# MasterVVK/qwen3-tts-axera-russian

Measured on AMD Instinct MI355X. Metric: 12Hz codec-tokens/s (codec frames/s, 16 codes each) + RTF, Qwen3-TTS-0.6B, higher is better.
Workload: dtype f16 weights/KV, f32 accumulate (talker+CP); vocoder exact fp32 (f32 MFMA); 1 GPU; configs[2]/[3]: batch=32 mixed ru/en prompts per GPU, 64 frames/utterance/step (prefill + hipGraph decode loop), utterance-sharded DP over 1 GPU(s); batch_per_gpu=32

## Files before the change

qwen3_tts_axera_russian_amd/build.py:

```python
from __future__ import annotations

import os
import shutil
import subprocess
import sys

HERE = os.path.dirname(os.path.abspath(__file__))
CSRC = os.path.join(HERE, "csrc")
LIB = os.path.join(HERE, "lib")
SOURCES = ["q3_common.cpp", "q3_formats.cpp", "q3_kernels.hip", "q3_model.hip", "q3_talker_api.hip", "q3_cp_api.hip",
           "q3_engine.hip", "q3_voc.hip", "q3_enc.hip", "q3_text_api.hip"]
TEST_SOURCES = ["q3_test_api.hip"]
ARCH = os.environ.get("Q3_OFFLOAD_ARCH", "gfx950")
EXTRA = os.environ.get("Q3_EXTRA_HIPCC_FLAGS", "-mllvm -amdgpu-kernarg-preload-count=16").split()


def _newer(dst: str, srcs) -> bool:
    if not os.path.exists(dst):
        return False
    t = os.path.getmtime(dst)
    return all(os.path.getmtime(s) <= t for s in srcs)


NO_SPILL = ("resunit_kernel", "linear_kernelILi1ELi1E", "linear_kernelILi1ELi2E", "linear_kernelILi2ELi1E",
            "linear_kernelILi2ELi2E", "attn_kernel", "attn_short_kernel", "cp_argmax_kernel", "talker_sample_kernel",
            "voc_attn_incr_kernel", "voc_incr_prepend_kernel", "voc_incr_emit_kernel")


def kernel_resources(lib_path: str):
    import re
    import struct
    import tempfile
    readelf = "/opt/rocm/lib/llvm/bin/llvm-readelf"
    d = open(lib_path, "rb").read()
    res = {}
    i = d.find(b"__CLANG_OFFLOAD_BUNDLE__")
    while i >= 0:
        n = struct.unpack_from("<Q", d, i + 24)[0]
        off = i + 32
        for _ in range(n):
            o, sz, ts = struct.unpack_from("<QQQ", d, off)
            off += 24
            triple = d[off:off + ts].decode()
            off += ts
            if ARCH in triple and sz:
                with tempfile.NamedTemporaryFile(suffix=".elf") as f:
                    f.write(d[i + o:i + o + sz])
                    f.flush()
# ... 85 lines not shown
```

qwen3_tts_axera_russian_amd/csrc/q3_cp.h:

```cpp
#pragma once
#include "q3_model.h"

namespace q3 {

struct CpFrameIO {
    int* codes = nullptr;
    const int* n_frames = nullptr;
    int frame_cap = 1;
    float* fb_h = nullptr;
    float* fb_ssq = nullptr;
    half_t* fb_xh = nullptr;
    const float* fb_gamma = nullptr;
    const float* pad_embed = nullptr;
    float temperature = 0.f;
    int top_k = 50;
    unsigned long long seed = 0;
    const unsigned long long* seed_ptr = nullptr;
    const int* forced = nullptr;
    const SlotParams* slots = nullptr;
};

int cp_seed_row0(const Work& w, int R, int row0 = 0, int R_total = 0);
int cp_frame(hipStream_t s, const Model& m, Work& w, KVCache& kv, int R, const CpFrameIO& io, int row0 = 0,
             int R_total = 0);

}
```

qwen3_tts_axera_russian_amd/csrc/q3_cp_api.hip:

```cpp
#include "../../include/qwen3tts_cp.h"
#include "q3_cp.h"

namespace q3 {

static bool two_row_enabled() {
    static const bool on = !(getenv("Q3_CP_TWO_ROW") && atoi(getenv("Q3_CP_TWO_ROW")) == 0);
    return on;
}

int cp_seed_row0(const Work& w, int R, int row0, int R_total) {
    (void)R;
    (void)row0;
    if (R_total <= 0) R_total = R;
    const int B16 = (R_total + 15) / 16 * 16;
    const bool two = two_row_enabled() && 2 * B16 <= w.max_rows;
    return two ? B16 : 0;
}

int cp_frame(hipStream_t s, const Model& m, Work& w, KVCache& kv, int R, const CpFrameIO& io, int row0, int R_total) {
    const ModelCfg& c = m.cfg;
    if (R_total <= 0) R_total = R;
    const int H = c.hidden, G = c.cp_groups;
    const int seed0 = cp_seed_row0(w, R, row0, R_total);
    RowMap rm;
    rm.slot_base = 0;
    rm.slot_stride = 1;
    rm.pos_stride = 0;
    if (seed0 > 0 && (row0 != 0 || R_total != R)) {
        RowMap r0;
        r0.slot_base = -seed0;
        r0.slot_stride = 1;
        r0.pos_base = 0;
        r0.pos_stride = 0;
        r0.same_slot_rows = true;
        if (run_stack(s, m, m.cp, w, kv, R, r0, 256, seed0 + row0)) return -1;
        if (launch_gather_embed(s, m.talker_emb, c.talker_vocab, H, io.codes, 0, io.n_frames, io.frame_cap, 0, w.h, w.ssq, R,
                                row0, R_total, io.forced, w.xh, m.cp.L[0].in_ln))
            return -1;
        RowMap r1 = rm;
        r1.pos_base = 1;
        r1.same_slot_rows = true;
        if (run_stack(s, m, m.cp, w, kv, R, r1, 256, row0)) return -1;
    } else if (seed0 > 0) {
        const int R16 = seed0;
        if (w.map_R16 != R16) {
            std::vector<int> slot(2 * R16), pos(2 * R16);
            for (int i = 0; i < 2 * R16; i++) {
                slot[i] = i % R16;
                pos[i] = i < R16 ? 1 : 0;
            }
            Q3_HIP(hipMemcpyAsync(w.map_slot, slot.data(), sizeof(int) * 2 * R16, hipMemcpyHostToDevice, s), -1);
            Q3_HIP(hipMemcpyAsync(w.map_pos, pos.data(), sizeof(int) * 2 * R16, hipMemcpyHostToDevice, s), -1);
            Q3_HIP(hipStreamSynchronize(s), -1);
            w.map_R16 = R16;
        }
        if (launch_gather_embed(s, m.talker_emb, c.talker_vocab, H, io.codes, 0, io.n_frames, io.frame_cap, 0, w.h, w.ssq, R,
                                row0, R_total, io.forced, w.xh, m.cp.L[0].in_ln))
            return -1;
        RowMap r2;
        r2.slot = w.map_slot;
        r2.pos = w.map_pos;
        r2.same_slot_rows = true;
        r2.valid_mod = R16;
        r2.valid_n = R;
        if (run_stack(s, m, m.cp, w, kv, R16 + R, r2, 256, 0)) return -1;
    } else {
        rm.pos_base = 0;
        if (run_stack(s, m, m.cp, w, kv, R, rm, 256, row0)) return -1;
        if (launch_gather_embed(s, m.talker_emb, c.talker_vocab, H, io.codes, 0, io.n_frames, io.frame_cap, 0, w.h, w.ssq, R,
                                row0, R_total, io.forced, w.xh, m.cp.L[0].in_ln))
            return -1;
        rm.pos_base = 1;
        if (run_stack(s, m, m.cp, w, kv, R, rm, 256, row0)) return -1;
    }
    const bool qkv_tab = m.cp_qkv_serves(R);
    for (int g = 0; g < G; g++) {
        if (g > 0) {
            rm.pos_base = g + 1;
            rm.skip_qkv0 = qkv_tab;
            if (run_stack(s, m, m.cp, w, kv, R, rm, 256, row0)) return -1;
        }
        LinArgs a;
        a.wp = m.cp_head[g].wp;
        a.N = c.cp_vocab;
        a.K = H;
        a.M = row0 + R;
        a.m_begin = row0;
// ... 234 lines not shown
```

qwen3_tts_axera_russian_amd/csrc/q3_engine.hip:

```cpp
#include "../../include/qwen3tts_engine.h"
#include "q3_cp.h"

#include <algorithm>
#include <chrono>
#include <cmath>

using namespace q3;

namespace {

struct Engine {
    Model* m = nullptr;
    int max_batch = 0, n_ctx = 0, max_frames = 0;
    hipStream_t s = nullptr;
    KVCache kv_t, kv_c;
    Work wt, wc;
    int prefill_rows = 0;
    int *d_slot = nullptr, *d_pos = nullptr;
    int* d_tiles = nullptr;
    int *d_iota = nullptr;
    int *d_past = nullptr, *d_npast = nullptr, *d_ntext = nullptr, *d_done = nullptr, *d_nframes = nullptr;
    int *d_pos0 = nullptr, *d_posdec = nullptr, *d_lastrow = nullptr;
    int* d_codes = nullptr;
    int* d_forced = nullptr;
// ... 72 lines not shown
    sa.R = R;
    sa.row0 = row0;
    sa.R_total = e->B;
    sa.audio_vocab = m.cfg.cp_vocab;
    sa.eos = m.cfg.codec_eos;
    sa.past = e->d_past;
    sa.n_past = e->d_npast;
    sa.n_text = e->d_ntext;
    sa.done = e->d_done;
    sa.codes = e->d_codes;
    sa.n_frames = e->d_nframes;
    sa.frame_cap = e->max_frames;
    sa.pos0 = e->d_pos0;
    sa.pos = e->d_posdec;
    sa.ignore_eos = e->ignore_eos;
    sa.max_frames = e->cap_frames;
    sa.temperature = e->t_temp;
    sa.top_k = e->t_top_k;
    sa.top_p = e->t_top_p;
    sa.seed = e->seed;
    sa.seed_ptr = e->d_seed;
    sa.forced = e->forced_on ? e->d_forced : nullptr;
    sa.slots = e->slot_mode ? e->d_slots : nullptr;
    if (launch_talker_sample(st, sa)) return -1;
    CpFrameIO io;
    io.codes = e->d_codes;
    io.n_frames = e->d_nframes;
    io.frame_cap = e->max_frames;
    io.fb_h = e->wt.h;
    io.fb_ssq = e->wt.ssq;
    io.fb_xh = e->wt.xh;
    io.fb_gamma = m.talker.L[0].in_ln;
    io.pad_embed = e->d_pad;
    io.temperature = e->c_temp;
    io.top_k = e->c_top_k;
    io.seed = e->seed ^ 0x5851F42D4C957F2Dull;
    io.seed_ptr = e->d_seed;
    io.forced = e->forced_on ? e->d_forced : nullptr;
    io.slots = e->slot_mode ? e->d_slots : nullptr;
    if (cp_frame(st, m, e->wc, e->kv_c, R, io, row0, e->B)) return -1;
    RowMap rm;
    rm.slot_base = 0;
    rm.slot_stride = 1;
    rm.pos = e->d_posdec;
    rm.rows_total = e->B;
    if (run_stack(st, m, m.talker, e->wt, e->kv_t, R, rm, 1024, row0)) return -1;
    return talker_tail(e, st, row0, R);
}

int n_chains_eff(const Engine* e) {
    const int nc = e->n_chains < 1 ? 1 : e->n_chains;
    return (nc > 1 && e->B % (16 * nc) == 0) ? nc : 1;
}

void chain_rows(const Engine* e, int c, int& row0, int& R) {
    const int nc = n_chains_eff(e);
    row0 = 0;
    for (int i = 0; i < c; i++) row0 += e->B / nc + (i < e->B % nc ? 1 : 0);
    R = e->B / nc + (c < e->B % nc ? 1 : 0);
}

bool make_stream(const Engine* e, hipStream_t* st) {
// ... 20 lines not shown
        chain_rows(e, c, row0, R);
        if (frame_chain(e, chain_stream(e, c), row0, R)) return -1;
    }
    return 0;
}

int fork_chains(Engine* e) {
    const int nc = n_chains_eff(e);
    if (nc == 1) return 0;
    Q3_HIP(hipEventRecord(e->ev_fork, e->s), -1);
    for (int c = 0; c < nc; c++) Q3_HIP(hipStreamWaitEvent(e->cs[c], e->ev_fork, 0), -1);
    return 0;
}
int join_chains(Engine* e) {
    const int nc = n_chains_eff(e);
    if (nc == 1) return 0;
    for (int c = 0; c < nc; c++) {
        Q3_HIP(hipEventRecord(e->ev_join[c], e->cs[c]), -1);
        Q3_HIP(hipStreamWaitEvent(e->s, e->ev_join[c], 0), -1);
    }
    return 0;
}

}

extern "C" {

void q3e_free(void* ee) {
    Engine* e = (Engine*)ee;
    if (!e) return;
    if (e->s) hipStreamSynchronize(e->s);
    for (auto& g : e->graph) g.reset();
    kv_free(e->kv_t);
    kv_free(e->kv_c);
    work_free(e->wt);
    work_free(e->wc);
    void* ps[] = {e->d_tiles, e->d_slot, e->d_pos,  e->d_iota,   e->d_past,    e->d_npast, e->d_ntext, e->d_done,
                  e->d_nframes, e->d_pos0, e->d_posdec, e->d_lastrow, e->d_codes, e->d_pad, e->d_forced, e->d_seed, e->d_slots};
    for (void* p : ps)
        if (p) hipFree(p);
    if (e->h_done) hipHostFree(e->h_done);
    if (e->h_read) hipHostFree(e->h_read);
    for (int c = 0; c < 8; c++) {
        if (e->cs[c]) hipStreamDestroy(e->cs[c]);
        if (e->ev_join[c]) hipEventDestroy(e->ev_join[c]);
    }
// ... 597 lines not shown
```

qwen3_tts_axera_russian_amd/csrc/q3_kernels.h:

```cpp
#pragma once
#include "q3_common.h"

namespace q3 {

enum { PRO_F16 = 0, PRO_NORM = 1 };
enum { EPI_STORE = 0, EPI_RESID = 1, EPI_SWIGLU = 2 };

struct LinArgs {
    int tl_node = -1;
    const half_t* wp = nullptr;
    int N = 0, K = 0, M = 0;
    int m_begin = 0;
    int swap_grid = 0;
    int nt = 0;
    const half_t* x16 = nullptr;
    const float* ssq = nullptr;
    int ssq_parts = 0;
    float eps = 1e-6f;
    float* y = nullptr;
    int ldy = 0;
    float* h_out = nullptr;
    float* ssq_out = nullptr;
    half_t* xh_out = nullptr;
    const float* gamma = nullptr;
// ... 7 lines not shown

enum { ATTN_FUSED = 0, ATTN_PREP = 1, ATTN_ATTEND = 2 };
struct AttnArgs {
    int tl_node = -1;
    float* qkv = nullptr;
    int ld = 0, R = 0, row0 = 0;
    const float* q_norm = nullptr;
    const float* k_norm = nullptr;
    float eps = 1e-6f;
    const float* rope_cos = nullptr;
    const float* rope_sin = nullptr;
    const int* slot = nullptr;
    const int* pos = nullptr;
    int slot_base = 0, slot_stride = 0, pos_base = 0, pos_stride = 0;
    half_t* kc = nullptr;
    half_t* vc = nullptr;
    int n_ctx = 0, n_kv = 0, n_heads = 0;
    half_t* out = nullptr;
    float scale = 0.f;
    int threads = 256;
    int valid_mod = 0, valid_n = 0;
    const int* tiles = nullptr;
    int n_tiles = 0;
};
int launch_attn(hipStream_t s, const AttnArgs& a, int mode);

int launch_ssq_rows(hipStream_t s, const float* rows, float* h, float* ssq, int R, int H, half_t* xh = nullptr,
                    const float* gamma = nullptr, int dst_row0 = 0);

struct FinalNormArgs {
    int tl_node = -1;
    const float* h = nullptr;
    const float* ssq = nullptr;
    int ssq_parts = 0;
    const float* gamma = nullptr;
    float eps = 1e-6f;
    int R = 0, H = 0, row0 = 0;
    const int* row_map = nullptr;
    int src_off = 0;
    float* out_f32 = nullptr;
    half_t* out_f16 = nullptr;
    float* out_copy = nullptr;
    float* out_copy_ssq = nullptr;
    int out_copy_row_off = 0;
    half_t* out_copy_xh = nullptr;
    const float* out_copy_gamma = nullptr;
};
int launch_final_norm(hipStream_t s, const FinalNormArgs& a);
// ... 17 lines not shown
struct TalkerSampleArgs {
    int tl_node = -1;
    const float* logits = nullptr;
    int V = 0, R = 0, row0 = 0, R_total = 0;
    int audio_vocab = 2048, eos = 2150;
    int* past = nullptr;
    int* n_past = nullptr;
    const int* n_text = nullptr;
    int* done = nullptr;
    int* codes = nullptr;
    int* n_frames = nullptr;
    int frame_cap = 0;
    const int* pos0 = nullptr;
    int* pos = nullptr;
    int ignore_eos = 0;
    int max_frames = 0;
    float rep_penalty = 1.2f;
    float temperature = 0.f, top_p = 0.95f;
    int top_k = 50;
    unsigned long long seed = 0;
    const unsigned long long* seed_ptr = nullptr;
    const int* forced = nullptr;
    const SlotParams* slots = nullptr;
};
int launch_talker_sample(hipStream_t s, const TalkerSampleArgs& a);

struct CpArgmaxArgs {
    int tl_node = -1;
    const float* logits = nullptr;
    int V = 0, R = 0, H = 0, row0 = 0, R_total = 0;
    int group = 0;
    int* codes = nullptr;
    const int* n_frames = nullptr;
    int frame_cap = 0;
    const float* next_table = nullptr;
    float* h_out = nullptr;
    float* ssq_out = nullptr;
    half_t* xh_out = nullptr;
    const float* gamma_next = nullptr;
    const float* next_qkv = nullptr;
    float* qkv_out = nullptr;
    int qkv_ld = 0;
    const float* talker_emb = nullptr;
    int talker_vocab = 0;
    const float* const* cp_tables = nullptr;
    const float* pad_embed = nullptr;
// ... 18 lines not shown
```

qwen3_tts_axera_russian_amd/csrc/q3_kernels.hip:

```cpp
#include "q3_kernels.h"

namespace q3 {

typedef _Float16 h8 __attribute__((ext_vector_type(8)));
typedef float f4 __attribute__((ext_vector_type(4)));

#ifdef Q3_TIMELINE
__device__ unsigned long long* g_tl = nullptr;
__device__ unsigned int g_tl_idx = 0;
__device__ unsigned int g_tl_cap = 0;
__device__ int g_skip = 0;
__device__ unsigned long long* g_ph = nullptr;
struct TlScope {
    unsigned int slot = 0xffffffffu;
    int id;
    __device__ __forceinline__ TlScope(int id_) : id(id_) {
        if (blockIdx.x == 0 && blockIdx.y == 0 && threadIdx.x == 0 && g_tl) {
            slot = atomicAdd(&g_tl_idx, 1u);
            if (slot < g_tl_cap) g_tl[2 * slot] = (wall_clock64() << 8) | (unsigned)id;
        }
    }
    __device__ __forceinline__ ~TlScope() {
        if (slot < g_tl_cap) g_tl[2 * slot + 1] = wall_clock64();
    }
};
__device__ unsigned long long* g_tl2 = nullptr;
__device__ int* g_tl2_kind = nullptr;
constexpr int TL2_MAXB = 1024;
struct TlScope2 {
    unsigned long long t0;
    int node, kind;
    __device__ __forceinline__ TlScope2(int n, int k) : node(n), kind(k) { t0 = wall_clock64(); }
    __device__ __forceinline__ ~TlScope2() {
        if (g_tl2 && node >= 0 && threadIdx.x == 0) {
            const unsigned b = blockIdx.x + gridDim.x * blockIdx.y;
            if (b < TL2_MAXB) {
                g_tl2[((size_t)node * TL2_MAXB + b) * 2] = t0;
                g_tl2[((size_t)node * TL2_MAXB + b) * 2 + 1] = wall_clock64();
            }
            if (b == 0 && g_tl2_kind) g_tl2_kind[node] = kind;
        }
    }
};
#define Q3_TL(id)      \
    if (g_skip) return; \
    TlScope2 tl_scope2_(a.tl_node, id); \
    TlScope tl_scope_(id)
#define Q3_PH(n)                                                                                       \
    do {                                                                                               \
        if (tl_scope_.slot < g_tl_cap && g_ph) g_ph[(size_t)tl_scope_.slot * 8 + (n)] = wall_clock64(); \
    } while (0)
#else
#ifndef Q3_WAVE_PRIO
#define Q3_WAVE_PRIO 3
#endif
#if Q3_WAVE_PRIO > 0
#define Q3_TL(id) __builtin_amdgcn_s_setprio(Q3_WAVE_PRIO)
#else
#define Q3_TL(id)
#endif
#define Q3_PH(n)
#endif

#define Q3_FETCH_ARGS(...) asm volatile("" ::__VA_ARGS__)

__device__ __forceinline__ int uniform_load(const int* p) {
    return *(const __attribute__((address_space(4))) int*)p;
}

__device__ __forceinline__ float wave_sum(float v) {
#pragma unroll
    for (int o = 32; o > 0; o >>= 1) v += __shfl_xor(v, o, 64);
    return v;
}
__device__ __forceinline__ float wave_max(float v) {
#pragma unroll
    for (int o = 32; o > 0; o >>= 1) v = fmaxf(v, __shfl_xor(v, o, 64));
    return v;
}
__device__ __forceinline__ half_t sat_half(float x) {
    return (half_t)fminf(fmaxf(x, -65504.f), 65504.f);
}
constexpr float NORM_PRE = 0.0625f, NORM_POST = 16.0f;
// ... 1165 lines not shown
#pragma unroll
    for (int e4 = 0; e4 < NE; e4 += 4) {
        const float4 t4 = *(const float4*)(&sc[hh][e4]);
        sv[e4] = t4.x;
        sv[e4 + 1] = t4.y;
        sv[e4 + 2] = t4.z;
        sv[e4 + 3] = t4.w;
    }
    float m = -INFINITY;
#pragma unroll
    for (int e = 0; e < NE; e++) m = fmaxf(m, e <= T ? sv[e] : -INFINITY);
    float L = 0.f, o = 0.f;
#pragma unroll
    for (int e = 0; e < NE; e++) {
        const float p = e <= T ? __expf(sv[e] - m) : 0.f;
        const float vf = e <= T ? (float)vs[e][d] : 0.f;
        L += p;
        o += p * vf;
    }
    Q3_PH(3);
    a.out[frag_idx(r, (2 * g + hh) * D + d, a.n_heads * D)] = sat_half(o / L);
}

__global__ void __launch_bounds__(256) attn_tile_mfma_kernel(AttnArgs a) {
    constexpr int D = 128, QP = 136, VP = 72, CH = 64;
    constexpr float LO = 2048.0f, ILO = 1.0f / 2048.0f;
    Q3_TL(35);
    const int g = blockIdx.y, tid = threadIdx.x, lane = tid & 63, w = tid >> 6;
    const int c = lane & 15, q4 = lane >> 4;
    int row0, nrows, slot, pos0;
    if (a.tiles) {
        const int4 t = *(const int4*)(a.tiles + 4 * blockIdx.x);
        row0 = t.x; nrows = t.y; slot = t.z; pos0 = t.w;
    } else {
        row0 = a.row0 + blockIdx.x * 16;
        nrows = a.R - blockIdx.x * 16 < 16 ? a.R - blockIdx.x * 16 : 16;
        slot = a.slot_base;
        pos0 = a.pos_base + blockIdx.x * 16;
    }
    extern __shared__ __attribute__((aligned(16))) char smem[];
    half_t* qh = (half_t*)smem;
    half_t* ql = qh + 32 * QP;
    half_t* ks = ql + 32 * QP;
    half_t* vs = ks + CH * QP;
    half_t* ph = vs + CH * QP;
    half_t* pl = ph + 32 * VP;
// ... 192 lines not shown
        return 0;
    }
    int threads = a.threads;
    const int fit = 65536 / (a.R * a.n_kv);
    if (threads > fit) threads = fit / 64 * 64;
    if (threads < 256) threads = 256;
    if (threads > 1024) threads = 1024;
    const size_t lds = ((size_t)(threads / 64) * (4 + 2 * 128)) * sizeof(float);
    AttnArgs a2 = a;
    a2.tl_node = tl_next_node();
    dim3 grid(a.R, a.n_kv);
#define Q3_ATTN(MODE_)                                                                                   \
    {                                                                                                    \
        if (threads <= 256)                                                                              \
            hipLaunchKernelGGL((attn_kernel<MODE_, 8>), grid, dim3(256), mode == ATTN_PREP ? 0 : lds, s, a2); \
        else                                                                                             \
            hipLaunchKernelGGL((attn_kernel<MODE_, 4>), grid, dim3(mode == ATTN_PREP ? 256 : threads),   \
                               mode == ATTN_PREP ? 0 : lds, s, a2);                                      \
    }
    if (mode == ATTN_FUSED) Q3_ATTN(ATTN_FUSED)
    else if (mode == ATTN_PREP) Q3_ATTN(ATTN_PREP)
    else Q3_ATTN(ATTN_ATTEND)
#undef Q3_ATTN
    Q3_HIP(hipGetLastError(), -1);
    return 0;
}

__device__ __forceinline__ void block_argmax(float& v, int& idx, float* sv, int* si) {
#pragma unroll
    for (int o = 32; o > 0; o >>= 1) {
        const float ov = __shfl_xor(v, o, 64);
        const int oi = __shfl_xor(idx, o, 64);
        if (ov > v || (ov == v && oi < idx)) {
            v = ov;
            idx = oi;
        }
    }
    const int w = threadIdx.x >> 6, nw = blockDim.x >> 6;
    if ((threadIdx.x & 63) == 0) {
        sv[w] = v;
        si[w] = idx;
    }
    __syncthreads();
    v = sv[0];
    idx = si[0];
    for (int i = 1; i < nw; i++)
// ... 160 lines not shown
    __syncthreads();
    return chosen;
}

__device__ __forceinline__ SlotParams uniform_slot(const SlotParams* p, int r) {
    static_assert(sizeof(SlotParams) % 4 == 0, "SlotParams is read as words");
    constexpr int NW = (int)(sizeof(SlotParams) / 4);
    const __attribute__((address_space(4))) int* q = (const __attribute__((address_space(4))) int*)(p + r);
    int w[NW];
#pragma unroll
    for (int i = 0; i < NW; i++) w[i] = q[i];
    SlotParams sp;
    __builtin_memcpy(&sp, w, sizeof(sp));
    return sp;
}

template <bool SLOTS>
__device__ __forceinline__ void talker_sample_row(const TalkerSampleArgs& a) {
    Q3_TL(42);
    __shared__ float sv[16];
    __shared__ int si[16];
    __shared__ int win[32];
    __shared__ int nwin;
    const int r = a.row0 + blockIdx.x;
    const int RT = a.R_total > 0 ? a.R_total : a.R;
    const int np = uniform_load(a.n_past + r);
    const int nt = uniform_load(a.n_text + r);
    const bool was_done = uniform_load(a.done + r) != 0;
    float temperature = a.temperature, top_p = a.top_p;
    int top_k = a.top_k, max_frames = a.max_frames;
    if constexpr (SLOTS) {
        const SlotParams sp = uniform_slot(a.slots, r);
        temperature = sp.t_temp;
        top_p = sp.t_top_p;
        top_k = sp.t_top_k;
        max_frames = sp.max_frames;
    }
    if (threadIdx.x == 0) nwin = np < 30 ? np : 30;
    if (threadIdx.x < 30 && threadIdx.x < np) {
        win[threadIdx.x] = a.past[r * 32 + ((np - 1 - threadIdx.x) & 31)];
    }
    __syncthreads();
    double progress = 0.0;
    float boost = 0.f;
    bool force_eos = false;
    if (nt > 0) {
// ... 44 lines not shown
        if (bidx >= a.V) bidx = a.eos;
    }
    if (threadIdx.x == 0) {
        int code = bidx;
        if (force_eos && !a.ignore_eos) code = a.eos;
        bool fin = was_done || code == a.eos || code >= a.audio_vocab || (max_frames > 0 && np >= max_frames);
        const int f = a.n_frames[r];
        if (!SLOTS || !fin || f <= a.frame_cap) a.n_frames[r] = f + 1;
        const bool keep = f < a.frame_cap;
        int* fc = a.codes + ((size_t)(keep ? f : 0) * RT + r) * 16;
        int used = code;
        if (a.forced && keep && !fin) {
            const int fz = a.forced[((size_t)f * RT + r) * 16];
            if (fz >= 0) used = fz;
        }
        if (fin || !keep) {
            a.done[r] = 1;
            if (keep) fc[0] = -1;
        } else {
            fc[0] = code;
            a.past[r * 32 + (np & 31)] = used;
            a.n_past[r] = np + 1;
            a.pos[r] = a.pos0[r] + np;
        }
    }
}
__global__ void talker_sample_kernel(TalkerSampleArgs a) { talker_sample_row<false>(a); }
__global__ void talker_sample_kernel_slots(TalkerSampleArgs a) { talker_sample_row<true>(a); }

static size_t sample_lds_bytes_slots(int n) { return (size_t)sample_sort_len(n) * 8; }

int launch_talker_sample(hipStream_t s, const TalkerSampleArgs& a) {
    if (a.R <= 0) return 0;
    if (a.slots && a.V > SAMPLE_SORT_CAP) {
        Q3_LOG("talker_sample: a vocabulary of %d is beyond the per-slot sampler (sort cap %d)", a.V, SAMPLE_SORT_CAP);
        return -1;
    }
    if (a.temperature > 1e-6f && effective_top_k(a.top_k, a.V) > SAMPLE_SEL_CAP && a.V > SAMPLE_SORT_CAP) {
        Q3_LOG("talker_sample: top_k=%d over a vocabulary of %d is beyond the device sampler (sort cap %d)", a.top_k, a.V,
               SAMPLE_SORT_CAP);
        return -1;
    }
    const size_t lds = a.slots ? sample_lds_bytes_slots(a.V) : sample_lds_bytes(a.V, a.top_k, a.temperature);
    TalkerSampleArgs a2 = a;
    a2.tl_node = tl_next_node();
    if (a.slots) hipLaunchKernelGGL(talker_sample_kernel_slots, dim3(a.R), dim3(256), lds, s, a2);
// ... 304 lines not shown
```

qwen3_tts_axera_russian_amd/csrc/q3_model.h:

```cpp
#pragma once
#include "q3_kernels.h"

namespace q3 {

struct DevLinear {
    half_t* wp = nullptr;
    int N = 0, K = 0;
};

struct DevLayer {
    DevLinear qkv, o, gu, down;
    float *in_ln = nullptr, *post_ln = nullptr, *q_norm = nullptr, *k_norm = nullptr;
};

struct DevStack {
    std::vector<DevLayer> L;
    float* final_norm = nullptr;
    const float* tail_gamma = nullptr;
    int ffn = 0;
    int nt = 0;
    size_t weight_bytes = 0;
};

struct Model {
// ... 43 lines not shown
    float *h = nullptr, *ssq = nullptr, *qkv = nullptr;
    half_t* xh = nullptr;
    half_t *attn = nullptr, *act = nullptr;
    float* hidden_f32 = nullptr;
    half_t* hidden_f16 = nullptr;
    float* logits = nullptr;
    int *map_slot = nullptr, *map_pos = nullptr;
    int map_R16 = 0;
};
int work_alloc(Work& w, const ModelCfg& c, int max_rows, int ffn, int max_vocab, hipStream_t s = nullptr);
void work_free(Work& w);
int work_zero(hipStream_t s, Work& w, const ModelCfg& c, int ffn, int max_vocab);

struct RowMap {
    const int* slot = nullptr;
    const int* pos = nullptr;
    int slot_base = 0, slot_stride = 0, pos_base = 0, pos_stride = 0;
    bool same_slot_rows = false;
    int valid_mod = 0, valid_n = 0;
    const int* tiles = nullptr;
    int n_tiles = 0;
    bool skip_qkv0 = false;
    int rows_total = 0;
};

int run_stack(hipStream_t s, const Model& m, const DevStack& st, Work& w, KVCache& kv, int R,
              const RowMap& rm, int attn_threads, int row0 = 0);

struct GraphExec {
    hipGraph_t g = nullptr;
    hipGraphExec_t e = nullptr;
    void reset();
};

}
```

qwen3_tts_axera_russian_amd/csrc/q3_model.hip:

```cpp
#include "q3_model.h"

#include <cmath>

namespace q3 {

namespace {

struct Loader {
    Model* m;
    const Pack& p;
    hipStream_t s = nullptr;
    half_t* stage = nullptr;
    size_t stage_elems = 0;
    std::vector<uint16_t> host16;
    bool ok = true;

    bool up(void* d, const void* src, size_t bytes) {
        return hipMemcpyAsync(d, src, bytes, hipMemcpyHostToDevice, s) == hipSuccess && hipStreamSynchronize(s) == hipSuccess;
    }
    void* dalloc(size_t bytes) {
        void* d = nullptr;
        if (hipMalloc(&d, bytes) != hipSuccess) {
            Q3_LOG("hipMalloc(%zu) failed", bytes);
            ok = false;
// ... 383 lines not shown
        t.rope_cos = m.rope_cos;
        t.rope_sin = m.rope_sin;
        t.slot = rm.slot;
        t.pos = rm.pos;
        t.slot_base = rm.slot_base;
        t.slot_stride = rm.slot_stride;
        t.pos_base = rm.pos_base;
        t.pos_stride = rm.pos_stride;
        t.kc = kv.k + li * kv.layer_stride();
        t.vc = kv.v + li * kv.layer_stride();
        t.n_ctx = kv.n_ctx;
        t.n_kv = c.n_kv;
        t.n_heads = c.n_heads;
        t.out = w.attn;
        t.scale = 1.0f / sqrtf((float)D);
        t.threads = attn_threads;
        if (rm.rows_total > R) {
            const int fit = 65536 / (rm.rows_total * c.n_kv);
            if (t.threads > fit) t.threads = fit / 64 * 64;
            if (t.threads < 256) t.threads = 256;
        }
        t.valid_mod = rm.valid_mod;
        t.valid_n = rm.valid_n;
        if (rm.same_slot_rows && R > 1) {
            if (launch_attn(s, t, ATTN_PREP)) return -1;
            if (rm.tiles && rm.n_tiles > 0) {
                t.tiles = rm.tiles;
                t.n_tiles = rm.n_tiles;
            } else if (!rm.slot && !rm.pos && rm.slot_stride == 0 && rm.pos_stride == 1 && rm.valid_mod == 0) {
                t.tiles = nullptr;
                t.n_tiles = (R + 15) / 16;
            }
            if (launch_attn(s, t, ATTN_ATTEND)) return -1;
        } else {
            if (launch_attn(s, t, ATTN_FUSED)) return -1;
        }
        a = LinArgs();
        a.wp = L.o.wp;
        a.N = H;
        a.K = L.o.K;
        a.M = row0 + R;
        a.m_begin = row0;
        a.nt = st.nt;
        a.x16 = w.attn;
        a.h_out = w.h;
        a.ssq_out = w.ssq;
        a.xh_out = w.xh;
// ... 41 lines not shown
```

qwen3_tts_axera_russian_amd/csrc/q3_test_api.hip:

```cpp
#include "q3_model.h"
#include "q3_voc_ops.h"
#include <chrono>
#include <cstring>
#include <vector>

using namespace q3;

namespace q3 {
int set_linear_tuning(int K, int mt16, int kbw);
int set_linear_split_rows(int on);
int set_linear_narrow8(int on);
int set_linear_wide_tiles(int on);
int set_attn_short(int on);
int set_gemm_min_rows(int n);
int set_gemm_glds(int on);
int reset_linear_knobs();
const char* last_linear_variant();
}

namespace {
struct DBuf {
    void* p = nullptr;
    ~DBuf() {
        if (p) hipFree(p);
    }
    bool alloc(size_t n) { return hipMalloc(&p, n ? n : 16) == hipSuccess; }
    bool up(const void* src, size_t n) { return alloc(n) && (n == 0 || hipMemcpy(p, src, n, hipMemcpyHostToDevice) == hipSuccess); }
};
}

extern "C" {

int q3t_set_linear_tuning(int K, int mt16, int kbw) { return set_linear_tuning(K, mt16, kbw); }
int q3t_set_linear_split_rows(int on) { return set_linear_split_rows(on); }
int q3t_set_linear_narrow8(int on) { return set_linear_narrow8(on); }
int q3t_set_linear_wide_tiles(int on) { return set_linear_wide_tiles(on); }
int q3t_set_attn_short(int on) { return set_attn_short(on); }
int q3t_set_gemm_min_rows(int n) { return set_gemm_min_rows(n); }
int q3t_set_gemm_glds(int on) { return set_gemm_glds(on); }
int q3t_reset_linear_knobs() { return reset_linear_knobs(); }
const char* q3t_last_linear_variant() { return last_linear_variant(); }

int q3t_linear(int M, int N, int K, const uint16_t* W, int gateup, int pro, int epi, const uint16_t* x16,
               const float* h, const float* gamma, float eps, float* y_or_h_io, float* ssq_out, uint16_t* act_out,
               int nt) {
    hipStream_t s = nullptr;
    const int Mp = (M + 127) / 128 * 128;
    DBuf dW, dWp, dx, dhrows, dh, dssq, dg, dy, dso, dact, dxh;
    if (!dW.up(W, (size_t)N * K * 2) || !dWp.alloc((size_t)N * K * 2)) return -1;
    if (gateup) {
        if (launch_pack_linear(s, (const half_t*)dW.p, N / 2, K, (half_t*)dWp.p, 0, 2)) return -1;
        if (launch_pack_linear(s, (const half_t*)dW.p + (size_t)(N / 2) * K, N / 2, K, (half_t*)dWp.p, 1, 2)) return -1;
    } else {
        if (launch_pack_linear(s, (const half_t*)dW.p, N, K, (half_t*)dWp.p, 0, 1)) return -1;
    }
    LinArgs a;
    a.wp = (const half_t*)dWp.p;
    a.N = N;
    a.K = K;
    a.M = M;
// ... 172 lines not shown
                const uint32_t v = hs[(size_t)m * (N / 16) + p];
                if (inside(m)) memcpy(&ssq_out[(size_t)m * (N / 16) + p], &v, 4);
                else if (v != GUARD32) outside++;
            }
        }
    } else {
        Q3_HIP(hipMemcpy(ha.data(), dact.p, ha.size() * 2, hipMemcpyDeviceToHost), -1);
        for (int m = 0; m < Mp; m++)
            for (int j = 0; j < NA; j++) {
                const uint16_t v = ha[frag_idx_host(m, j, NA)];
                if (inside(m)) act[(size_t)m * NA + j] = v;
                else if (v != GUARD16) outside++;
            }
    }
    return outside ? -3 : 0;
}

int q3t_attn(int mode, int R, int row0, const float* qkv, const float* q_norm, const float* k_norm, float eps,
             const float* rope_cos, const float* rope_sin, int max_pos, const int* slot, const int* pos, int slot_base,
             int slot_stride, int pos_base, int pos_stride, uint16_t* kc, uint16_t* vc, int n_slots, int n_ctx,
             const int* tiles, int n_tiles, int valid_mod, int valid_n, int threads, uint16_t* out) {
    constexpr int NH = 16, NKV = 8, D = 128, LD = (NH + 2 * NKV) * D, OW = NH * D;
    constexpr uint16_t GUARD = 0x7d5au;
    if (mode != 0 && mode != 1) return -2;
    if (R <= 0 || row0 < 0 || !qkv || !q_norm || !k_norm || !rope_cos || !rope_sin || !kc || !vc || !out) return -2;
    if (max_pos <= 0 || n_slots <= 0 || n_ctx <= 0 || threads < 64 || threads > 1024 || threads % 64) return -2;
    if (valid_mod < 0 || (valid_mod > 0 && (valid_n < 0 || valid_n > valid_mod))) return -2;
    const int rows = row0 + R;
    auto skipped = [&](int r) { return valid_mod > 0 && (r % valid_mod) >= valid_n; };
    auto row_slot = [&](int r) { return slot ? slot[r - row0] : slot_base + r * slot_stride; };
    auto row_pos = [&](int r) { return pos ? pos[r - row0] : pos_base + r * pos_stride; };
    for (int r = row0; r < rows; r++) {
        if (skipped(r)) continue;
        const int sl = row_slot(r), p = row_pos(r);
        if (sl < 0 || sl >= n_slots || p < 0 || p >= n_ctx || p >= max_pos) return -2;
    }
    if (mode == 0) {
        if (n_tiles != 0 || tiles) return -2;
        std::vector<char> seen((size_t)n_slots, 0);
        for (int r = row0; r < rows; r++) {
            if (skipped(r)) continue;
            if (seen[(size_t)row_slot(r)]++) return -2;
        }
    } else if (n_tiles > 0 && !tiles) {
        if (slot || pos || slot_stride != 0 || pos_stride != 1 || valid_mod != 0 || n_tiles != (R + 15) / 16) return -2;
    } else if (n_tiles > 0) {
        for (int i = 0; i < n_tiles; i++) {
            const int* t = tiles + 4 * i;
            if (t[0] < row0 || t[1] < 1 || t[1] > 16 || t[0] + t[1] > rows) return -2;
            if (t[2] < 0 || t[2] >= n_slots || t[3] < 0 || t[3] + t[1] > n_ctx) return -2;
        }
    } else if (n_tiles < 0 || tiles) {
        return -2;
    }
    hipStream_t s = nullptr;
    const int Rp = (rows + 15) / 16 * 16;
    const size_t cache = (size_t)n_slots * NKV * n_ctx * D;
    std::vector<float> hq((size_t)Rp * LD, 0.f);
    memcpy(hq.data() + (size_t)row0 * LD, qkv, (size_t)R * LD * 4);
    std::vector<uint16_t> ho((size_t)Rp * OW, GUARD);
// ... 17 lines not shown
    t.R = R;
    t.row0 = row0;
    t.q_norm = (const float*)dqn.p;
    t.k_norm = (const float*)dkn.p;
    t.eps = eps;
    t.rope_cos = (const float*)dcs.p;
    t.rope_sin = (const float*)dsn.p;
    t.slot = slot ? (const int*)dslot.p : nullptr;
    t.pos = pos ? (const int*)dpos.p : nullptr;
    t.slot_base = slot_base;
    t.slot_stride = slot_stride;
    t.pos_base = pos_base;
    t.pos_stride = pos_stride;
    t.kc = (half_t*)dkc.p;
    t.vc = (half_t*)dvc.p;
    t.n_ctx = n_ctx;
    t.n_kv = NKV;
    t.n_heads = NH;
    t.out = (half_t*)dout.p;
    t.scale = 1.0f / sqrtf((float)D);
    t.threads = threads;
    t.valid_mod = valid_mod;
    t.valid_n = valid_n;
    if (mode == 0) {
        if (launch_attn(s, t, ATTN_FUSED)) return -1;
    } else {
        if (launch_attn(s, t, ATTN_PREP)) return -1;
        t.tiles = tiles ? (const int*)dtiles.p : nullptr;
        t.n_tiles = n_tiles;
        if (launch_attn(s, t, ATTN_ATTEND)) return -1;
    }
    Q3_HIP(hipDeviceSynchronize(), -1);
    Q3_HIP(hipMemcpy(kc, dkc.p, cache * 2, hipMemcpyDeviceToHost), -1);
    Q3_HIP(hipMemcpy(vc, dvc.p, cache * 2, hipMemcpyDeviceToHost), -1);
    Q3_HIP(hipMemcpy(ho.data(), dout.p, ho.size() * 2, hipMemcpyDeviceToHost), -1);
    for (int r = row0; r < rows; r++)
        for (int k = 0; k < OW; k++) out[(size_t)(r - row0) * OW + k] = ho[frag_idx_host(r, k, OW)];
    for (int r = 0; r < Rp; r++) {
        if (r >= row0 && r < rows) continue;
        for (int k = 0; k < OW; k++)
            if (ho[frag_idx_host(r, k, OW)] != GUARD) return -3;
    }
    return 0;
}

int q3t_voc_attn(int kernel, const float* x, float* y, int B, int H, int D, int L, int window, float theta) {
    constexpr float GUARD = 1234.5f;
// ... 244 lines not shown
```

Baseline: 10130 codec_frames/s.

## Fuse code-0 embedding into talker sampler and add paired two-position CP attention

Moves the code-0 embedding gather for the code predictor into the talker sampling kernel, so a separate gather launch is skipped when the seed row is ahead. It also adds a specialised attention kernel that handles the CP's first two positions (row and its paired row) in one launch, replacing the separate prep and attend attention launches for that stage. Both are gated by Q3_FRAME_FOLDS, which is on by default. The aim is fewer kernel launches and graph nodes per frame. The cost is extra per-block work in the sampler and a hand-written softmax path that must match the reference numerics.

```diff
diff --git a/qwen3_tts_axera_russian_amd/build.py b/qwen3_tts_axera_russian_amd/build.py
--- a/qwen3_tts_axera_russian_amd/build.py
+++ b/qwen3_tts_axera_russian_amd/build.py
@@ -23,7 +23,7 @@
 
 
 NO_SPILL = ("resunit_kernel", "linear_kernelILi1ELi1E", "linear_kernelILi1ELi2E", "linear_kernelILi2ELi1E",
-            "linear_kernelILi2ELi2E", "attn_kernel", "attn_short_kernel", "cp_argmax_kernel", "talker_sample_kernel",
+            "linear_kernelILi2ELi2E", "attn_kernel", "attn_short_kernel", "attn_pair_kernel", "cp_argmax_kernel", "talker_sample_kernel",
             "voc_attn_incr_kernel", "voc_incr_prepend_kernel", "voc_incr_emit_kernel")
 
 
diff --git a/qwen3_tts_axera_russian_amd/csrc/q3_cp.h b/qwen3_tts_axera_russian_amd/csrc/q3_cp.h
--- a/qwen3_tts_axera_russian_amd/csrc/q3_cp.h
+++ b/qwen3_tts_axera_russian_amd/csrc/q3_cp.h
@@ -18,7 +18,10 @@
     const unsigned long long* seed_ptr = nullptr;
     const int* forced = nullptr;
     const SlotParams* slots = nullptr;
+    bool code0_embedded = false;
 };
+
+bool frame_folds_enabled();
 
 int cp_seed_row0(const Work& w, int R, int row0 = 0, int R_total = 0);
 int cp_frame(hipStream_t s, const Model& m, Work& w, KVCache& kv, int R, const CpFrameIO& io, int row0 = 0,
diff --git a/qwen3_tts_axera_russian_amd/csrc/q3_cp_api.hip b/qwen3_tts_axera_russian_amd/csrc/q3_cp_api.hip
--- a/qwen3_tts_axera_russian_amd/csrc/q3_cp_api.hip
+++ b/qwen3_tts_axera_russian_amd/csrc/q3_cp_api.hip
@@ -5,6 +5,11 @@
 
 static bool two_row_enabled() {
     static const bool on = !(getenv("Q3_CP_TWO_ROW") && atoi(getenv("Q3_CP_TWO_ROW")) == 0);
+    return on;
+}
+
+bool frame_folds_enabled() {
+    static const bool on = !(getenv("Q3_FRAME_FOLDS") && atoi(getenv("Q3_FRAME_FOLDS")) == 0);
     return on;
 }
 
@@ -22,6 +27,10 @@
     if (R_total <= 0) R_total = R;
     const int H = c.hidden, G = c.cp_groups;
     const int seed0 = cp_seed_row0(w, R, row0, R_total);
+    if (io.code0_embedded && seed0 == 0) {
+        Q3_LOG("cp_frame: position 1's rows cannot be written ahead of the sequential form");
+        return -1;
+    }
     RowMap rm;
     rm.slot_base = 0;
     rm.slot_stride = 1;
@@ -34,7 +43,8 @@
         r0.pos_stride = 0;
         r0.same_slot_rows = true;
         if (run_stack(s, m, m.cp, w, kv, R, r0, 256, seed0 + row0)) return -1;
-        if (launch_gather_embed(s, m.talker_emb, c.talker_vocab, H, io.codes, 0, io.n_frames, io.frame_cap, 0, w.h, w.ssq, R,
+        if (!io.code0_embedded &&
+            launch_gather_embed(s, m.talker_emb, c.talker_vocab, H, io.codes, 0, io.n_frames, io.frame_cap, 0, w.h, w.ssq, R,
                                 row0, R_total, io.forced, w.xh, m.cp.L[0].in_ln))
             return -1;
         RowMap r1 = rm;
@@ -54,7 +64,8 @@
             Q3_HIP(hipStreamSynchronize(s), -1);
             w.map_R16 = R16;
         }
-        if (launch_gather_embed(s, m.talker_emb, c.talker_vocab, H, io.codes, 0, io.n_frames, io.frame_cap, 0, w.h, w.ssq, R,
+        if (!io.code0_embedded &&
+            launch_gather_embed(s, m.talker_emb, c.talker_vocab, H, io.codes, 0, io.n_frames, io.frame_cap, 0, w.h, w.ssq, R,
                                 row0, R_total, io.forced, w.xh, m.cp.L[0].in_ln))
             return -1;
         RowMap r2;
@@ -63,6 +74,7 @@
         r2.same_slot_rows = true;
         r2.valid_mod = R16;
         r2.valid_n = R;
+        if (frame_folds_enabled()) r2.pair_off = R16;
         if (run_stack(s, m, m.cp, w, kv, R16 + R, r2, 256, 0)) return -1;
     } else {
         rm.pos_base = 0;
diff --git a/qwen3_tts_axera_russian_amd/csrc/q3_engine.hip b/qwen3_tts_axera_russian_amd/csrc/q3_engine.hip
--- a/qwen3_tts_axera_russian_amd/csrc/q3_engine.hip
+++ b/qwen3_tts_axera_russian_amd/csrc/q3_engine.hip
@@ -118,6 +118,16 @@
     sa.seed_ptr = e->d_seed;
     sa.forced = e->forced_on ? e->d_forced : nullptr;
     sa.slots = e->slot_mode ? e->d_slots : nullptr;
+    const bool embed_code0 = frame_folds_enabled() && cp_seed_row0(e->wc, R, row0, e->B) > 0;
+    if (embed_code0) {
+        sa.emb_table = m.talker_emb;
+        sa.emb_vocab = m.cfg.talker_vocab;
+        sa.emb_H = m.cfg.hidden;
+        sa.emb_h = e->wc.h;
+        sa.emb_ssq = e->wc.ssq;
+        sa.emb_xh = e->wc.xh;
+        sa.emb_gamma = m.cp.L[0].in_ln;
+    }
     if (launch_talker_sample(st, sa)) return -1;
     CpFrameIO io;
     io.codes = e->d_codes;
@@ -134,6 +144,7 @@
     io.seed_ptr = e->d_seed;
     io.forced = e->forced_on ? e->d_forced : nullptr;
     io.slots = e->slot_mode ? e->d_slots : nullptr;
+    io.code0_embedded = embed_code0;
     if (cp_frame(st, m, e->wc, e->kv_c, R, io, row0, e->B)) return -1;
     RowMap rm;
     rm.slot_base = 0;
@@ -200,6 +211,18 @@
     return 0;
 }
 
+}
+
+namespace q3 {
+int engine_graph_nodes(void* ee) {
+    Engine* e = (Engine*)ee;
+    size_t total = 0;
+    for (int c = 0; e && c < 8; c++) {
+        size_t n = 0;
+        if (e->graph[c].g && hipGraphGetNodes(e->graph[c].g, nullptr, &n) == hipSuccess) total += n;
+    }
+    return (int)total;
+}
 }
 
 extern "C" {
diff --git a/qwen3_tts_axera_russian_amd/csrc/q3_kernels.h b/qwen3_tts_axera_russian_amd/csrc/q3_kernels.h
--- a/qwen3_tts_axera_russian_amd/csrc/q3_kernels.h
+++ b/qwen3_tts_axera_russian_amd/csrc/q3_kernels.h
@@ -53,8 +53,10 @@
     int valid_mod = 0, valid_n = 0;
     const int* tiles = nullptr;
     int n_tiles = 0;
+    int pair_off = 0;
 };
 int launch_attn(hipStream_t s, const AttnArgs& a, int mode);
+int launch_attn_pair(hipStream_t s, const AttnArgs& a);
 
 int launch_ssq_rows(hipStream_t s, const float* rows, float* h, float* ssq, int R, int H, half_t* xh = nullptr,
                     const float* gamma = nullptr, int dst_row0 = 0);
@@ -118,6 +120,12 @@
     const unsigned long long* seed_ptr = nullptr;
     const int* forced = nullptr;
     const SlotParams* slots = nullptr;
+    const float* emb_table = nullptr;
+    int emb_vocab = 0, emb_H = 0;
+    float* emb_h = nullptr;
+    float* emb_ssq = nullptr;
+    half_t* emb_xh = nullptr;
+    const float* emb_gamma = nullptr;
 };
 int launch_talker_sample(hipStream_t s, const TalkerSampleArgs& a);
 
diff --git a/qwen3_tts_axera_russian_amd/csrc/q3_kernels.hip b/qwen3_tts_axera_russian_amd/csrc/q3_kernels.hip
--- a/qwen3_tts_axera_russian_amd/csrc/q3_kernels.hip
+++ b/qwen3_tts_axera_russian_amd/csrc/q3_kernels.hip
@@ -4,6 +4,15 @@
 
 typedef _Float16 h8 __attribute__((ext_vector_type(8)));
 typedef float f4 __attribute__((ext_vector_type(4)));
+
+#ifndef Q3_WAVE_PRIO
+#define Q3_WAVE_PRIO 3
+#endif
+#if Q3_WAVE_PRIO > 0
+#define Q3_PRIO_RAISE() __builtin_amdgcn_s_setprio(Q3_WAVE_PRIO)
+#else
+#define Q3_PRIO_RAISE()
+#endif
 
 #ifdef Q3_TIMELINE
 __device__ unsigned long long* g_tl = nullptr;
@@ -44,6 +53,7 @@
 };
 #define Q3_TL(id)      \
     if (g_skip) return; \
+    Q3_PRIO_RAISE();    \
     TlScope2 tl_scope2_(a.tl_node, id); \
     TlScope tl_scope_(id)
 #define Q3_PH(n)                                                                                       \
@@ -51,14 +61,7 @@
         if (tl_scope_.slot < g_tl_cap && g_ph) g_ph[(size_t)tl_scope_.slot * 8 + (n)] = wall_clock64(); \
     } while (0)
 #else
-#ifndef Q3_WAVE_PRIO
-#define Q3_WAVE_PRIO 3
-#endif
-#if Q3_WAVE_PRIO > 0
-#define Q3_TL(id) __builtin_amdgcn_s_setprio(Q3_WAVE_PRIO)
-#else
-#define Q3_TL(id)
-#endif
+#define Q3_TL(id) Q3_PRIO_RAISE()
 #define Q3_PH(n)
 #endif
 
@@ -1270,6 +1273,146 @@
     a.out[frag_idx(r, (2 * g + hh) * D + d, a.n_heads * D)] = sat_half(o / L);
 }
 
+struct AttnPart {
+    float m, l, a;
+};
+__device__ __forceinline__ AttnPart attn_part_one(float s, float vf) {
+    const float n = fmaxf(-INFINITY, s);
+    const float c = __expf(-INFINITY - n), p = __expf(s - n);
+    return {n, 0.f * c + p, 0.f * c + p * vf};
+}
+__device__ __forceinline__ AttnPart attn_part_merge(const AttnPart& x, const AttnPart& y) {
+    const float n = fmaxf(x.m, y.m);
+    const float c = (x.m == -INFINITY) ? 0.f : __expf(x.m - n), d = (y.m == -INFINITY) ? 0.f : __expf(y.m - n);
+    return {n, x.l * c + y.l * d, x.a * c + y.a * d};
+}
+__device__ __forceinline__ float attn_part_finish(const AttnPart& x, const AttnPart& y) {
+    const AttnPart none = {-INFINITY, 0.f, 0.f};
+    const AttnPart w0 = attn_part_merge(attn_part_merge(x, y), none);
+    const float M = fmaxf(-INFINITY, w0.m);
+    const float c = (w0.m == -INFINITY) ? 0.f : __expf(w0.m - M);
+    float L = 0.f, o = 0.f;
+    L += w0.l * c;
+    o += w0.a * c;
+    return o / L;
+}
+__global__ void __launch_bounds__(256)
+    attn_pair_kernel(float* __restrict__ p_qkv, int p_ld, int p_row0, int p_n_heads, int p_n_kv,
+                     const float* __restrict__ p_q_norm, const float* __restrict__ p_k_norm,
+                     const float* __restrict__ p_rope_cos, const float* __restrict__ p_rope_sin, int p_pair_off,
+                     int p_slot_base, AttnArgs a) {
+    constexpr int D = 128;
+    a.qkv = p_qkv;
+    a.ld = p_ld;
+    a.row0 = p_row0;
+    a.n_heads = p_n_heads;
+    a.n_kv = p_n_kv;
+    a.q_norm = p_q_norm;
+    a.k_norm = p_k_norm;
+    a.rope_cos = p_rope_cos;
+    a.rope_sin = p_rope_sin;
+    a.pair_off = p_pair_off;
+    a.slot_base = p_slot_base;
+    Q3_FETCH_ARGS("s"(a.eps), "s"(a.slot_stride), "s"(a.kc), "s"(a.vc), "s"(a.n_ctx), "s"(a.out), "s"(a.scale));
+    Q3_TL(34);
+    const int g = blockIdx.y;
+    const int tid = threadIdx.x, lane = tid & 63, w = tid >> 6;
+    const int r1 = a.row0 + blockIdx.x, r0 = r1 + a.pair_off;
+    const int rp[2] = {r0, r1};
+    const int slot = a.slot_base + r1 * a.slot_stride;
+    __shared__ float qs[2][2][D];
+    __shared__ float kn[2][D];
+    __shared__ __attribute__((aligned(16))) half_t vs[2][D];
+    __shared__ float sc[2][2][2];
+    const size_t cbase = ((size_t)slot * a.n_kv + g) * (size_t)a.n_ctx * D;
+    const int l16 = tid & 15, grp = tid >> 4;
+    const int hh = tid >> 7, d = tid & 127;
+    float x0[2], x1[2], gm0 = 1.f, gm1 = 1.f, cs[2] = {1.f, 1.f}, sn[2] = {0.f, 0.f};
+    const int col0 = w < 2 ? (2 * g + w) * D : w == 2 ? (a.n_heads + g) * D : (a.n_heads + a.n_kv + g) * D;
+#pragma unroll
+    for (int p = 0; p < 2; p++) {
+        const float* src = a.qkv + (size_t)rp[p] * a.ld + col0;
+        x0[p] = src[lane];
+        x1[p] = src[lane + 64];
+    }
+    if (w < 3) {
+        const float* gam = w < 2 ? a.q_norm : a.k_norm;
+        gm0 = gam[lane];
+        gm1 = gam[lane + 64];
+#pragma unroll
+        for (int p = 0; p < 2; p++) {
+            cs[p] = a.rope_cos[p * 64 + lane];
+            sn[p] = a.rope_sin[p * 64 + lane];
+        }
+    }
+    __builtin_amdgcn_sched_barrier(0);
+    Q3_PH(0);
+#pragma unroll
+    for (int p = 0; p < 2; p++) {
+        float y0 = x0[p], y1 = x1[p];
+        if (w < 3) {
+            float ss = wave_sum(y0 * y0 + y1 * y1);
+            const float iv = 1.0f / sqrtf(ss / (float)D + a.eps);
+            y0 = (y0 * iv) * gm0;
+            y1 = (y1 * iv) * gm1;
+            const float z0 = y0 * cs[p] - y1 * sn[p];
+            const float z1 = y1 * cs[p] + y0 * sn[p];
+            y0 = z0;
+            y1 = z1;
+        }
+        if (w < 2) {
+            qs[p][w][lane] = y0;
+            qs[p][w][lane + 64] = y1;
+        } else {
+            const half_t h0 = sat_half(y0), h1 = sat_half(y1);
+            half_t* cd = (w == 2 ? a.kc : a.vc) + cbase + (size_t)p * D;
+            cd[lane] = h0;
+            cd[lane + 64] = h1;
+            if (w == 2) {
+                kn[p][lane] = (float)h0;
+                kn[p][lane + 64] = (float)h1;
+            } else {
+                vs[p][lane] = h0;
+                vs[p][lane + 64] = h1;
+            }
+        }
+    }
+    __syncthreads();
+    Q3_PH(1);
+    if (grp < 3) {
+        const int p = grp > 0, e = grp == 2;
+        float d0 = 0.f, d1 = 0.f;
+        {
+#pragma clang fp contract(off)
+#pragma unroll
+            for (int j = 0; j < 8; j++) {
+                const float kf = kn[e][l16 * 8 + j];
+                const float t0 = (qs[p][0][l16 * 8 + j] * a.scale) * kf, t1 = (qs[p][1][l16 * 8 + j] * a.scale) * kf;
+                d0 = d0 + t0;
+                d1 = d1 + t1;
+            }
+        }
+#pragma unroll
+        for (int o = 8; o > 0; o >>= 1) {
+            d0 += __shfl_xor(d0, o, 16);
+            d1 += __shfl_xor(d1, o, 16);
+        }
+        if (l16 == 0) {
+            sc[p][0][e] = d0;
+            sc[p][1][e] = d1;
+        }
+    }
+    __syncthreads();
+    Q3_PH(2);
+    const float v0 = (float)vs[0][d], v1 = (float)vs[1][d];
+    const AttnPart none = {-INFINITY, 0.f, 0.f};
+    const float o0 = attn_part_finish(attn_part_one(sc[0][hh][0], v0), none);
+    const float o1 = attn_part_finish(attn_part_one(sc[1][hh][0], v0), attn_part_one(sc[1][hh][1], v1));
+    Q3_PH(3);
+    a.out[frag_idx(r0, (2 * g + hh) * D + d, a.n_heads * D)] = sat_half(o0);
+    a.out[frag_idx(r1, (2 * g + hh) * D + d, a.n_heads * D)] = sat_half(o1);
+}
+
 __global__ void __launch_bounds__(256) attn_tile_mfma_kernel(AttnArgs a) {
     constexpr int D = 128, QP = 136, VP = 72, CH = 64;
     constexpr float LO = 2048.0f, ILO = 1.0f / 2048.0f;
@@ -1508,6 +1651,24 @@
     else if (mode == ATTN_PREP) Q3_ATTN(ATTN_PREP)
     else Q3_ATTN(ATTN_ATTEND)
 #undef Q3_ATTN
+    Q3_HIP(hipGetLastError(), -1);
+    return 0;
+}
+
+int launch_attn_pair(hipStream_t s, const AttnArgs& a) {
+    if (a.R <= 0) return 0;
+    if (a.n_heads != 2 * a.n_kv) {
+        Q3_LOG("attn: only GQA group 2 (16q/8kv) is built, got %d/%d", a.n_heads, a.n_kv);
+        return -1;
+    }
+    if (a.pair_off < a.R || a.n_ctx < 2) {
+        Q3_LOG("attn_pair: pair_off=%d rows=%d n_ctx=%d", a.pair_off, a.R, a.n_ctx);
+        return -1;
+    }
+    AttnArgs a2 = a;
+    a2.tl_node = tl_next_node();
+    hipLaunchKernelGGL(attn_pair_kernel, dim3(a.R, a.n_kv), dim3(256), 0, s, a2.qkv, a2.ld, a2.row0, a2.n_heads, a2.n_kv,
+                       a2.q_norm, a2.k_norm, a2.rope_cos, a2.rope_sin, a2.pair_off, a2.slot_base, a2);
     Q3_HIP(hipGetLastError(), -1);
     return 0;
 }
@@ -1714,6 +1875,7 @@
     __shared__ int si[16];
     __shared__ int win[32];
     __shared__ int nwin;
+    __shared__ int emb_tok;
     const int r = a.row0 + blockIdx.x;
     const int RT = a.R_total > 0 ? a.R_total : a.R;
     const int np = uniform_load(a.n_past + r);
@@ -1804,6 +1966,23 @@
             a.past[r * 32 + (np & 31)] = used;
             a.n_past[r] = np + 1;
             a.pos[r] = a.pos0[r] + np;
+        }
+        int tok = fin ? -1 : used;
+        if (!keep) {
+            const size_t last = ((size_t)(a.frame_cap - 1) * RT + r) * 16;
+            tok = a.codes[last];
+            if (a.forced && a.forced[last] >= 0 && tok >= 0) tok = a.forced[last];
+        }
+        emb_tok = tok;
+    }
+    if (a.emb_table) {
+        __syncthreads();
+        const int t = emb_tok;
+        const bool ok = t >= 0 && t < a.emb_vocab;
+        for (int k4 = threadIdx.x; k4 < a.emb_H / 4; k4 += blockDim.x) {
+            float4 v = make_float4(0.f, 0.f, 0.f, 0.f);
+            if (ok) v = *(const float4*)(a.emb_table + (size_t)t * a.emb_H + k4 * 4);
+            store_row_ssq(a.emb_h, a.emb_ssq, r, a.emb_H, k4, v, a.emb_xh, a.emb_gamma);
         }
     }
 }
diff --git a/qwen3_tts_axera_russian_amd/csrc/q3_model.h b/qwen3_tts_axera_russian_amd/csrc/q3_model.h
--- a/qwen3_tts_axera_russian_amd/csrc/q3_model.h
+++ b/qwen3_tts_axera_russian_amd/csrc/q3_model.h
@@ -89,6 +89,7 @@
     int n_tiles = 0;
     bool skip_qkv0 = false;
     int rows_total = 0;
+    int pair_off = 0;
 };
 
 int run_stack(hipStream_t s, const Model& m, const DevStack& st, Work& w, KVCache& kv, int R,
diff --git a/qwen3_tts_axera_russian_amd/csrc/q3_model.hip b/qwen3_tts_axera_russian_amd/csrc/q3_model.hip
--- a/qwen3_tts_axera_russian_amd/csrc/q3_model.hip
+++ b/qwen3_tts_axera_russian_amd/csrc/q3_model.hip
@@ -429,7 +429,13 @@
         }
         t.valid_mod = rm.valid_mod;
         t.valid_n = rm.valid_n;
-        if (rm.same_slot_rows && R > 1) {
+        if (rm.pair_off > 0) {
+            t.R = rm.valid_n;
+            t.pair_off = rm.pair_off;
+            t.slot_base = 0;
+            t.slot_stride = 1;
+            if (launch_attn_pair(s, t)) return -1;
+        } else if (rm.same_slot_rows && R > 1) {
             if (launch_attn(s, t, ATTN_PREP)) return -1;
             if (rm.tiles && rm.n_tiles > 0) {
                 t.tiles = rm.tiles;
diff --git a/qwen3_tts_axera_russian_amd/csrc/q3_test_api.hip b/qwen3_tts_axera_russian_amd/csrc/q3_test_api.hip
--- a/qwen3_tts_axera_russian_amd/csrc/q3_test_api.hip
+++ b/qwen3_tts_axera_russian_amd/csrc/q3_test_api.hip
@@ -16,6 +16,7 @@
 int set_gemm_glds(int on);
 int reset_linear_knobs();
 const char* last_linear_variant();
+int engine_graph_nodes(void* e);
 }
 
 namespace {
@@ -36,6 +37,7 @@
 int q3t_set_linear_narrow8(int on) { return set_linear_narrow8(on); }
 int q3t_set_linear_wide_tiles(int on) { return set_linear_wide_tiles(on); }
 int q3t_set_attn_short(int on) { return set_attn_short(on); }
+int q3t_engine_graph_nodes(void* e) { return engine_graph_nodes(e); }
 int q3t_set_gemm_min_rows(int n) { return set_gemm_min_rows(n); }
 int q3t_set_gemm_glds(int on) { return set_gemm_glds(on); }
 int q3t_reset_linear_knobs() { return reset_linear_knobs(); }
@@ -254,7 +256,7 @@
              const int* tiles, int n_tiles, int valid_mod, int valid_n, int threads, uint16_t* out) {
     constexpr int NH = 16, NKV = 8, D = 128, LD = (NH + 2 * NKV) * D, OW = NH * D;
     constexpr uint16_t GUARD = 0x7d5au;
-    if (mode != 0 && mode != 1) return -2;
+    if (mode != 0 && mode != 1 && mode != 2) return -2;
     if (R <= 0 || row0 < 0 || !qkv || !q_norm || !k_norm || !rope_cos || !rope_sin || !kc || !vc || !out) return -2;
     if (max_pos <= 0 || n_slots <= 0 || n_ctx <= 0 || threads < 64 || threads > 1024 || threads % 64) return -2;
     if (valid_mod < 0 || (valid_mod > 0 && (valid_n < 0 || valid_n > valid_mod))) return -2;
@@ -267,7 +269,12 @@
         const int sl = row_slot(r), p = row_pos(r);
         if (sl < 0 || sl >= n_slots || p < 0 || p >= n_ctx || p >= max_pos) return -2;
     }
-    if (mode == 0) {
+    if (mode == 2) {
+        if (n_tiles != 0 || tiles || row0 != 0 || valid_mod <= 0 || valid_n < 1 || R != valid_mod + valid_n || !slot || !pos)
+            return -2;
+        for (int r = 0; r < R; r++)
+            if (!skipped(r) && (slot[r] != r % valid_mod || pos[r] != (r < valid_mod ? 1 : 0))) return -2;
+    } else if (mode == 0) {
         if (n_tiles != 0 || tiles) return -2;
         std::vector<char> seen((size_t)n_slots, 0);
         for (int r = row0; r < rows; r++) {
@@ -331,7 +338,13 @@
     t.threads = threads;
     t.valid_mod = valid_mod;
     t.valid_n = valid_n;
-    if (mode == 0) {
+    if (mode == 2) {
+        t.R = valid_n;
+        t.pair_off = valid_mod;
+        t.slot_base = 0;
+        t.slot_stride = 1;
+        if (launch_attn_pair(s, t)) return -1;
+    } else if (mode == 0) {
         if (launch_attn(s, t, ATTN_FUSED)) return -1;
     } else {
         if (launch_attn(s, t, ATTN_PREP)) return -1;
```

Result: no change. 10180 codec_frames/s (median of 6 runs) (+0.6%).
